# monahand1023/imageclust

Measured on AMD Instinct MI355X. Metric: images/sec (embed+Ward), higher is better.
Workload: dtype bf16; 1 GPU; the metric's size (configs[2]'s N=100000) on 1 GPU: 100000 synthetic 224x224x3 images (structured, seed 20250217; 100000 on this rank), ResNet50-v1 bf16 batch=256 -> 2048-d pooled E -> Ward min=5 max=50 (merge loop on GPU0) -> cluster ids on host; n_images_total=100000, embed_dim=2048, weights=synthetic seed 1, device=AMD Radeon Graphics (gfx950:sramecc+:xnack-)

## Files before the change

imageclust_amd/csrc/conv_p8.h:

```cpp
#pragma once
#include "mfma_tile.h"
#include "resnet_fused.h"

template <int MW, int NWV>
struct p8_geom {
    static_assert(MW * NWV == 8 && (NWV == 4 || NWV == 2), "8 waves");
    static constexpr int BM = MW * 128, BN = NWV * 64;
    static constexpr int PX = MW, PW = NWV / 2;
    static constexpr int SX = PX * 8192, SW = PW * 8192;
    static constexpr int O_WA = 0, O_XA = SW, O_WB = SW + SX, O_XB = 2 * SW + SX;
    static constexpr int BUF = 2 * (SW + SX);
    static constexpr int LDS = 2 * BUF;
    static constexpr int INFLIGHT = 2 * PW + PX;
    static_assert(INFLIGHT == 6 && LDS <= 160 * 1024, "counted vmcnt(6); the CU's 160 KiB");
};

template <int NP>
__device__ __forceinline__ void p8_dma(const i32x4_t &srd, const unsigned (&voff)[NP], unsigned soff, unsigned lds0)
{
    unsigned keep;
    if constexpr (NP == 1) {
        asm volatile("s_mov_b32 %0, m0\n\ts_mov_b32 m0, %4\n\ts_nop 4\n\tbuffer_load_dwordx4 %1, %2, %3 offen lds\n\ts_mov_b32 m0, %0"
                     : "=&s"(keep)
                     : "v"(voff[0]), "s"(srd), "s"(soff), "s"(lds0)
                     : "memory");
    } else if constexpr (NP == 2) {
        asm volatile("s_mov_b32 %0, m0\n\ts_mov_b32 m0, %5\n\ts_nop 4\n\tbuffer_load_dwordx4 %1, %3, %4 offen lds\n\t"
                     "s_mov_b32 m0, %6\n\ts_nop 0\n\tbuffer_load_dwordx4 %2, %3, %4 offen lds\n\ts_mov_b32 m0, %0"
                     : "=&s"(keep)
                     : "v"(voff[0]), "v"(voff[1]), "s"(srd), "s"(soff), "s"(lds0), "s"(lds0 + 0x2000u)
                     : "memory");
    } else {
        static_assert(NP == 4, "1, 2 or 4 pieces");
        asm volatile("s_mov_b32 %0, m0\n\ts_mov_b32 m0, %7\n\ts_nop 4\n\tbuffer_load_dwordx4 %1, %5, %6 offen lds\n\t"
                     "s_mov_b32 m0, %8\n\ts_nop 0\n\tbuffer_load_dwordx4 %2, %5, %6 offen lds\n\t"
                     "s_mov_b32 m0, %9\n\ts_nop 0\n\tbuffer_load_dwordx4 %3, %5, %6 offen lds\n\t"
                     "s_mov_b32 m0, %10\n\ts_nop 0\n\tbuffer_load_dwordx4 %4, %5, %6 offen lds\n\ts_mov_b32 m0, %0"
                     : "=&s"(keep)
                     : "v"(voff[0]), "v"(voff[1]), "v"(voff[2]), "v"(voff[3]), "s"(srd), "s"(soff), "s"(lds0), "s"(lds0 + 0x2000u), "s"(lds0 + 0x4000u),
                       "s"(lds0 + 0x6000u)
                     : "memory");
    }
}

template <int MW, int NWV, bool TAPS, bool DUAL, bool SPLIT = false, bool X3 = false>
__global__ __launch_bounds__(512) void conv_p8_kernel(const conv_args p)
{
    static_assert(!(SPLIT && DUAL), "the split form covers single-operand layers");
    static_assert(!(SPLIT && X3), "the split form is bf16 only");
    typedef p8_geom<MW, NWV> G;
    typedef unsigned u32x2_t __attribute__((ext_vector_type(2)));
    constexpr int PX = G::PX, PW = G::PW;
    __shared__ __attribute__((aligned(1024))) unsigned char smem[G::LDS];
    const int tid = threadIdx.x, lane = tid & 63;
    const int wid = __builtin_amdgcn_readfirstlane(tid >> 6);
    const int wr = wid / NWV, wc = wid % NWV;
    const int grp = wid >> 2;
    const int ntile = p.gx * p.gy;
    const int role = SPLIT ? (int)blockIdx.x / ntile : 0;
    const int tile = xcd_remap((int)blockIdx.x - role * ntile, ntile);
    const int m0 = (tile / p.gy) * G::BM, n0 = (tile % p.gy) * G::BN;
    const i32x4_t xsrd = bn56_srd(p.X, (unsigned)((size_t)p.B * p.H * p.W * p.Cin * 2));
    const i32x4_t wsrd = bn56_srd(p.Wt, (unsigned)((size_t)p.Cout * p.K * 2));
    const i32x4_t x2srd = DUAL ? bn56_srd(p.X2, (unsigned)((size_t)p.B * p.H2 * p.W2 * p.Cin2 * 2)) : xsrd;

    unsigned vx[2][PX], vw[2][PW], vx2[DUAL ? 2 : 1][PX], vmask[TAPS ? 2 : 1][PX];
#pragma unroll
    for (int j = 0; j < PX; ++j) {
        const int sr = (j * 8 + wid) * 8 + (lane >> 3);
        const unsigned ls16 = (unsigned)(((lane & 7) ^ ((sr >> 1) & 7)) << 4);
#pragma unroll
        for (int h = 0; h < 2; ++h) {
            const int m = m0 + (sr >> 6) * 128 + h * 64 + (sr & 63);
            const bool ok = (int64_t)m < p.M;
            const unsigned mm = ok ? (unsigned)m : 0u;
            const unsigned tq = mm / (unsigned)p.Wo;
            const int ox = (int)(mm - tq * (unsigned)p.Wo);
            const int b = (int)(tq / (unsigned)p.Ho);
            const int oy = (int)(tq - (unsigned)b * (unsigned)p.Ho);
            const int iy0 = oy * p.stride - p.pad, ix0 = ox * p.stride - p.pad;
            const unsigned off = (unsigned)((((b * p.H + iy0) * p.W + ix0) * p.Cin) * 2) + ls16;
            if (TAPS) {
                unsigned mk = 0;
                for (int kh = 0; kh < p.KH; ++kh)
                    for (int kw = 0; kw < p.KW; ++kw)
                        if (ok && (unsigned)(iy0 + kh) < (unsigned)p.H && (unsigned)(ix0 + kw) < (unsigned)p.W) mk |= 1u << (kh * p.KW + kw);
                vmask[h][j] = mk;
                vx[h][j] = off;
            } else {
                vx[h][j] = ok ? off : BN56_OOB;
            }
            if (DUAL) vx2[h][j] = ok ? (unsigned)((((b * p.H2 + oy * p.stride2) * p.W2 + ox * p.stride2) * p.Cin2) * 2) + ls16 : BN56_OOB;
        }
    }
#pragma unroll
    for (int j = 0; j < PW; ++j) {
        const int sr = (j * 8 + wid) * 8 + (lane >> 3);
        const unsigned ls16 = (unsigned)(((lane & 7) ^ ((sr >> 1) & 7)) << 4);
#pragma unroll
        for (int h = 0; h < 2; ++h) {
            const int wrow = n0 + (sr >> 5) * 64 + h * 32 + (sr & 31);
            vw[h][j] = (unsigned)wrow * (unsigned)p.K * 2u + ls16;
        }
    }
    const unsigned lds0 = __builtin_amdgcn_readfirstlane(lds_addr_of(smem) + wid * 1024);
    const int l15 = lane & 15, q = lane >> 4, fsw = (l15 >> 1) & 7;
    const unsigned char *xrd[2], *wrd[2];
#pragma unroll
    for (int s = 0; s < 2; ++s) {
        const int ph = ((4 * s + q) ^ fsw) << 4;
        xrd[s] = smem + (wr * 64 + l15) * 128 + ph;
        wrd[s] = smem + (wc * 32 + l15) * 128 + ph;
    }
    f32x4 acc[8][4];
#pragma unroll
    for (int i = 0; i < 8; ++i)
#pragma unroll
        for (int j = 0; j < 4; ++j) acc[i][j] = f32x4{0.f, 0.f, 0.f, 0.f};

    const int nt = SPLIT ? p.K / 128 : p.K / 64;
    const int kt0 = (SPLIT && role == 0) ? nt : 0;
    const int nt1 = (p.KH * p.KW * p.Cin) / 64;
    int xs_t = kt0, xs_ci = 0, xs_kw = 0, xs_kh = 0;
    unsigned xs_off = 0, xs_bit = 1;
    if (SPLIT && TAPS && kt0) {
        const int cpt = p.Cin / 64, tap = kt0 / cpt;
        xs_ci = (kt0 - tap * cpt) * 64;
        xs_kh = tap / p.KW;
        xs_kw = tap - xs_kh * p.KW;
        xs_bit = 1u << tap;
        xs_off = (unsigned)(((xs_kh * p.W + xs_kw) * p.Cin + xs_ci) * 2);
    }
    auto stage_w = [&](int h, int buf, int t) {
        p8_dma<PW>(wsrd, vw[h], (unsigned)(kt0 + t) * 128u, lds0 + buf * G::BUF + (h ? G::O_WB : G::O_WA));
    };
    auto stage_x = [&](int h, int buf) {
        const unsigned dst = lds0 + buf * G::BUF + (h ? G::O_XB : G::O_XA);
        if (DUAL && xs_t >= nt1) {
            p8_dma<PX>(x2srd, vx2[DUAL ? h : 0], (unsigned)(xs_t - nt1) * 128u, dst);
        } else if (TAPS) {
            unsigned v[PX];
#pragma unroll
            for (int j = 0; j < PX; ++j) v[j] = (vmask[TAPS ? h : 0][j] & xs_bit) ? vx[h][j] + xs_off : BN56_OOB;
            p8_dma<PX>(xsrd, v, 0u, dst);
        } else {
            p8_dma<PX>(xsrd, vx[h], (unsigned)xs_t * 128u, dst);
        }
        if (h == 1) {
            ++xs_t;
            if (TAPS) {
                xs_ci += 64;
                if (xs_ci == p.Cin) {
                    xs_ci = 0;
                    xs_bit <<= 1;
                    if (++xs_kw == p.KW) {
                        xs_kw = 0;
                        ++xs_kh;
                    }
                }
                xs_off = (unsigned)(((xs_kh * p.W + xs_kw) * p.Cin + xs_ci) * 2);
            }
        }
    };
    uint4 xf[4][2], w0[2][2], w1[2][2];
    auto mma = [&](int hx, int hw, uint4 (&wf)[2][2]) {
        __builtin_amdgcn_s_barrier();
        asm volatile("s_waitcnt lgkmcnt(0)" ::: "memory");
        __builtin_amdgcn_s_setprio(1);
        if constexpr (X3) {
#pragma unroll
            for (int u = 0; u < 3; ++u)
#pragma unroll
                for (int m = 0; m < 4; ++m)
#pragma unroll
                    for (int n = 0; n < 2; ++n) acc[hx * 4 + m][hw * 2 + n] = mfma16(wf[n][u == 1], xf[m][u == 2], acc[hx * 4 + m][hw * 2 + n]);
        } else {
#pragma unroll
            for (int s = 0; s < 2; ++s)
#pragma unroll
                for (int m = 0; m < 4; ++m)
#pragma unroll
                    for (int n = 0; n < 2; ++n) acc[hx * 4 + m][hw * 2 + n] = mfma16(wf[n][s], xf[m][s], acc[hx * 4 + m][hw * 2 + n]);
        }
        __builtin_amdgcn_s_setprio(0);
        __builtin_amdgcn_s_barrier();
    };
    auto ktile = [&](auto bufc, auto modec, int t) {
        constexpr int BUF = decltype(bufc)::value, MODE = decltype(modec)::value;
        const size_t bo = (size_t)BUF * G::BUF;
#pragma unroll
        for (int n = 0; n < 2; ++n)
#pragma unroll
            for (int s = 0; s < 2; ++s) w0[n][s] = *reinterpret_cast<const uint4 *>(wrd[s] + bo + G::O_WA + n * 2048);
        __builtin_amdgcn_sched_barrier(0);
#pragma unroll
        for (int m = 0; m < 4; ++m)
#pragma unroll
            for (int s = 0; s < 2; ++s) xf[m][s] = *reinterpret_cast<const uint4 *>(xrd[s] + bo + G::O_XA + m * 2048);
        if (MODE <= 1) stage_x(1, BUF ^ 1);
        asm volatile("s_waitcnt lgkmcnt(8)" ::: "memory");
        mma(0, 0, w0);
#pragma unroll
        for (int n = 0; n < 2; ++n)
#pragma unroll
            for (int s = 0; s < 2; ++s) w1[n][s] = *reinterpret_cast<const uint4 *>(wrd[s] + bo + G::O_WB + n * 2048);
        if (MODE == 0) stage_w(0, BUF, t + 2);
        mma(0, 1, w1);
#pragma unroll
        for (int m = 0; m < 4; ++m)
#pragma unroll
            for (int s = 0; s < 2; ++s) xf[m][s] = *reinterpret_cast<const uint4 *>(xrd[s] + bo + G::O_XB + m * 2048);
        if (MODE == 0) stage_x(0, BUF);
        mma(1, 1, w1);
        if (MODE == 0) {
            stage_w(1, BUF, t + 2);
            asm volatile("s_waitcnt vmcnt(6)" ::: "memory");
        } else if (MODE == 1) {
            asm volatile("s_waitcnt vmcnt(0)" ::: "memory");
        }
        mma(1, 0, w0);
    };
    stage_w(0, 0, 0);
    stage_x(0, 0);
    stage_w(1, 0, 0);
    stage_x(1, 0);
    stage_w(0, 1, 1);
    stage_x(0, 1);
    stage_w(1, 1, 1);
    asm volatile("s_waitcnt vmcnt(6)" ::: "memory");
    __builtin_amdgcn_s_barrier();
    if (grp == 1) __builtin_amdgcn_s_barrier();
    int t = 0;
    for (; t + 4 <= nt; t += 2) {
        ktile(std::integral_constant<int, 0>(), std::integral_constant<int, 0>(), t);
        ktile(std::integral_constant<int, 1>(), std::integral_constant<int, 0>(), t + 1);
    }
    ktile(std::integral_constant<int, 0>(), std::integral_constant<int, 1>(), t);
    ktile(std::integral_constant<int, 1>(), std::integral_constant<int, 2>(), t + 1);
    if (grp == 0) __builtin_amdgcn_s_barrier();

    if constexpr (SPLIT) {
        typedef unsigned u32x4_t __attribute__((ext_vector_type(4)));
        const __amdgpu_buffer_rsrc_t psrd = __builtin_amdgcn_make_buffer_rsrc(p.sk_part, 0, (int)((size_t)ntile * (32 * 512 * 16)), 0x00020000);
        const int voff = tid * 16;
        const int soff0 = tile * (32 * 512 * 16);
        if (role == 0) {
#pragma unroll
            for (int i = 0; i < 8; ++i)
#pragma unroll
                for (int j = 0; j < 4; ++j)
                    __builtin_amdgcn_raw_buffer_store_b128(__builtin_bit_cast(u32x4_t, acc[i][j]), psrd, voff, soff0 + (i * 4 + j) * 8192, 16 );
            asm volatile("s_waitcnt vmcnt(0)" ::: "memory");
            __syncthreads();
            if (tid == 0) __hip_atomic_store(p.sk_flag + tile, p.sk_epoch, __ATOMIC_RELAXED, __HIP_MEMORY_SCOPE_AGENT);
            return;
        }
        for (int spin = 0; spin < (1 << 22); ++spin) {
            if (__hip_atomic_load(p.sk_flag + tile, __ATOMIC_RELAXED, __HIP_MEMORY_SCOPE_AGENT) == p.sk_epoch) break;
            __builtin_amdgcn_s_sleep(2);
        }
        __builtin_amdgcn_fence(__ATOMIC_ACQUIRE, "wavefront");
#pragma unroll
        for (int g = 0; g < 4; ++g) {
            u32x4_t o[8];
#pragma unroll
            for (int k = 0; k < 8; ++k) o[k] = __builtin_amdgcn_raw_buffer_load_b128(psrd, voff, soff0 + (g * 8 + k) * 8192, 16 );
#pragma unroll
            for (int k = 0; k < 8; ++k) acc[(g * 8 + k) >> 2][(g * 8 + k) & 3] += __builtin_bit_cast(f32x4, o[k]);
        }
    }

    typedef uint16_t elem;
    elem *Yg = (elem *)p.Y;
    const elem *Rg = (const elem *)p.R;
    const int cbl = (q & 1) * 16 + (q >> 1) * 8;
    const int64_t yld = X3 ? 2 * (int64_t)p.Cout : (int64_t)p.Cout;
    auto ycol = [&](int c) { return X3 ? c + (c & ~31) : c; };
    float sc[2][8], sh[2][8];
#pragma unroll
    for (int i = 0; i < 2; ++i) {
        const int c = n0 + wc * 64 + i * 32 + cbl;
        const float4 a0 = *reinterpret_cast<const float4 *>(p.scale + c), a1 = *reinterpret_cast<const float4 *>(p.scale + c + 4);
        const float4 b0 = *reinterpret_cast<const float4 *>(p.shift + c), b1 = *reinterpret_cast<const float4 *>(p.shift + c + 4);
        sc[i][0] = a0.x; sc[i][1] = a0.y; sc[i][2] = a0.z; sc[i][3] = a0.w; sc[i][4] = a1.x; sc[i][5] = a1.y; sc[i][6] = a1.z; sc[i][7] = a1.w;
        sh[i][0] = b0.x; sh[i][1] = b0.y; sh[i][2] = b0.z; sh[i][3] = b0.w; sh[i][4] = b1.x; sh[i][5] = b1.y; sh[i][6] = b1.z; sh[i][7] = b1.w;
    }
#pragma unroll
    for (int hx = 0; hx < 2; ++hx) {
        uint4 rv[4][2], rl[2];
        if (Rg && !X3) {
#pragma unroll
            for (int m = 0; m < 4; ++m) {
                const int64_t mrow = (int64_t)m0 + wr * 128 + hx * 64 + m * 16 + l15;
#pragma unroll
                for (int i = 0; i < 2; ++i)
                    rv[m][i] = mrow < p.M ? *reinterpret_cast<const uint4 *>(Rg + mrow * p.Cout + n0 + wc * 64 + i * 32 + cbl) : make_uint4(0, 0, 0, 0);
            }
        }
#pragma unroll
        for (int m = 0; m < 4; ++m) {
            const int64_t mrow = (int64_t)m0 + wr * 128 + hx * 64 + m * 16 + l15;
            if (X3 && Rg) {
#pragma unroll
                for (int i = 0; i < 2; ++i) {
                    const elem *r = Rg + mrow * yld + ycol(n0 + wc * 64 + i * 32 + cbl);
                    rv[m][i] = mrow < p.M ? *reinterpret_cast<const uint4 *>(r) : make_uint4(0, 0, 0, 0);
                    rl[i] = mrow < p.M ? *reinterpret_cast<const uint4 *>(r + 32) : make_uint4(0, 0, 0, 0);
                }
            }
#pragma unroll
            for (int i = 0; i < 2; ++i) {
                const f32x4 ta = acc[hx * 4 + m][2 * i], tb = acc[hx * 4 + m][2 * i + 1];
                float v[8];
#pragma unroll
                for (int j = 0; j < 4; ++j) {
                    const u32x2_t r = __builtin_amdgcn_permlane16_swap(__float_as_uint(ta[j]), __float_as_uint(tb[j]), false, false);
                    v[j] = __uint_as_float(r[0]);
                    v[4 + j] = __uint_as_float(r[1]);
                }
#pragma unroll
                for (int e = 0; e < 8; ++e) v[e] = v[e] * sc[i][e] + sh[i][e];
                if (Rg) {
                    const elem *re = reinterpret_cast<const elem *>(&rv[m][i]);
                    if constexpr (X3) {
                        const elem *rle = reinterpret_cast<const elem *>(&rl[i]);
#pragma unroll
                        for (int e = 0; e < 8; ++e) v[e] += BF16::to_f(re[e]) + BF16::to_f(rle[e]);
                    } else {
#pragma unroll
                        for (int e = 0; e < 8; ++e) v[e] += BF16::to_f(re[e]);
                    }
                }
                if (p.relu) {
#pragma unroll
                    for (int e = 0; e < 8; ++e) v[e] = fmaxf(v[e], 0.0f);
                }
                uint4 ov, ol;
                elem *oe = reinterpret_cast<elem *>(&ov);
                if constexpr (X3) {
                    elem *ole = reinterpret_cast<elem *>(&ol);
#pragma unroll
                    for (int e = 0; e < 8; ++e) BF16X3::split(v[e], oe[e], ole[e]);
                } else {
#pragma unroll
                    for (int e = 0; e < 8; ++e) oe[e] = BF16::from_f(v[e]);
                }
                elem *yo = Yg + mrow * yld + ycol(n0 + wc * 64 + i * 32 + cbl);
                if (mrow < p.M) {
                    *reinterpret_cast<uint4 *>(yo) = ov;
                    if (X3) *reinterpret_cast<uint4 *>(yo + 32) = ol;
                }
            }
        }
    }
}

#ifndef P8_AUTO_MIN_NT
#define P8_AUTO_MIN_NT 4
#endif
static int conv_p8_layout(const conv_args &a) { return a.Cout % 256 == 0 ? 1 : (a.Cout % 128 == 0 ? 2 : 0); }
static bool conv_p8_eligible(const conv_args &a, int mode )
{
    if (mode == 0) return false;
    const int lay = conv_p8_layout(a);
    if (!lay || a.Cin % 64 || (a.X2 && a.Cin2 % 64)) return false;
    if (a.KH * a.KW > 9 || a.KH * a.KW * a.Cin + (a.X2 ? a.Cin2 : 0) != a.K) return false;
    if (a.X2 && (a.KH != 1 || a.KW != 1 || a.stride != 1 || a.pad != 0)) return false;
    const int nt = a.K / 64;
    if (a.K % 128) return false;
    if ((size_t)a.B * a.H * a.W * a.Cin * 2 >= (1ull << 31) || (size_t)a.Cout * a.K * 2 >= (1ull << 31)) return false;
    if (a.X2 && (size_t)a.B * a.H2 * a.W2 * a.Cin2 * 2 >= (1ull << 31)) return false;
    if (a.M >= (1ll << 31) - 512) return false;
    if (mode >= 2) return true;
    return nt >= P8_AUTO_MIN_NT;
}

static bool conv_p8_split_eligible(const icl_ctx *ctx, const conv_args &a)
{
    return ctx->conv_sk && !a.X2 && a.Ho * a.Wo <= 49 && a.K % 256 == 0 && a.K >= ctx->conv_sk_min_k && a.Cout % 256 == 0;
}
static int conv_p8_split_scratch(icl_ctx *ctx, hipStream_t strm, int tiles, conv_args &a)
{
    icl_sk_slot *sl = nullptr;
    for (auto &s : ctx->sk)
        if (s.part && s.stream == strm) sl = &s;
    if (!sl)
        for (auto &s : ctx->sk)
            if (!s.part && !sl) sl = &s;
    if (!sl) return ICL_ERR_NOMEM;
    if (sl->cap < tiles) {
        if (sl->part) {
            ICL_HIP(ctx, hipStreamSynchronize(strm));
            (void)hipFree(sl->part);
            (void)hipFree(sl->flag);
            sl->part = nullptr;
            sl->flag = nullptr;
            sl->cap = 0;
        }
        if (tiles > 4096) return ICL_ERR_UNSUPPORTED;
        const int cap = std::max(tiles, 128);
        ICL_HIP(ctx, hipMalloc(&sl->part, (size_t)cap * 32 * 512 * 16));
        ICL_HIP(ctx, hipMalloc((void **)&sl->flag, (size_t)cap * 4));
        ICL_HIP(ctx, hipMemsetAsync(sl->flag, 0, (size_t)cap * 4, strm));
        sl->cap = cap;
        sl->stream = strm;
        sl->epoch = 0;
    }
    a.sk_part = sl->part;
    a.sk_flag = sl->flag;
    a.sk_epoch = ++sl->epoch;
    return ICL_OK;
}

template <int MW, int NWV, bool X3>
static void launch_conv_p8_t(icl_ctx *ctx, conv_args &a)
{
    typedef p8_geom<MW, NWV> G;
    hipStream_t strm = ctx->cur_stream ? ctx->cur_stream : ctx->stream;
    a.gx = (int)icl_ceil_div(a.M, G::BM);
    a.gy = a.Cout / G::BN;
    const bool taps = a.KH * a.KW > 1 || a.pad != 0;
    if constexpr (NWV == 4 && !X3) {
        if (conv_p8_split_eligible(ctx, a) && conv_p8_split_scratch(ctx, strm, a.gx * a.gy, a) == ICL_OK) {
            const dim3 grid2((unsigned)(2 * a.gx * a.gy));
            if (taps) hipLaunchKernelGGL((conv_p8_kernel<MW, NWV, true, false, true>), grid2, dim3(512), 0, strm, a);
            else hipLaunchKernelGGL((conv_p8_kernel<MW, NWV, false, false, true>), grid2, dim3(512), 0, strm, a);
            ++ctx->conv_sk_launches;
            return;
        }
    }
    const dim3 grid((unsigned)(a.gx * a.gy));
    if (a.X2) hipLaunchKernelGGL((conv_p8_kernel<MW, NWV, false, true, false, X3>), grid, dim3(512), 0, strm, a);
    else if (taps) hipLaunchKernelGGL((conv_p8_kernel<MW, NWV, true, false, false, X3>), grid, dim3(512), 0, strm, a);
    else hipLaunchKernelGGL((conv_p8_kernel<MW, NWV, false, false, false, X3>), grid, dim3(512), 0, strm, a);
}
template <bool X3 = false>
static void launch_conv_p8(icl_ctx *ctx, conv_args &a)
{
    if (conv_p8_layout(a) == 1) launch_conv_p8_t<2, 4, X3>(ctx, a);
    else launch_conv_p8_t<4, 2, X3>(ctx, a);
}
```

imageclust_amd/csrc/distance_i8.hip:

```cpp
#include "icl_common.h"
#include "distance.h"
#include "mfma_tile.h"

#include <algorithm>
#include <cmath>
#include <type_traits>

typedef int di8_i32x4 __attribute__((ext_vector_type(4)));

#define DI8_OOB 0x80000000u
#define DI8_SLOT 16384
#define DI8_BUF 65536
#define DI8_WA 0
#define DI8_XA 1
#define DI8_WB 2
#define DI8_XB 3

__device__ __forceinline__ di8_i32x4 di8_srd(const void *base, unsigned bytes)
{
    const unsigned long long a = (unsigned long long)base;
    di8_i32x4 r;
    r.x = __builtin_amdgcn_readfirstlane((int)(unsigned)a);
    r.y = __builtin_amdgcn_readfirstlane((int)(unsigned)(a >> 32));
    r.z = __builtin_amdgcn_readfirstlane((int)bytes);
    r.w = 0x00020000;
    return r;
}
__device__ __forceinline__ void di8_dma2(const di8_i32x4 &srd, unsigned voff0, unsigned voff1, unsigned soff, unsigned lds0)
{
    unsigned keep;
    const unsigned lds1 = lds0 + 0x2000u;
    asm volatile("s_mov_b32 %0, m0\n\t"
                 "s_mov_b32 m0, %5\n\t"
                 "s_nop 4\n\t"
                 "buffer_load_dwordx4 %1, %3, %4 offen lds\n\t"
                 "s_mov_b32 m0, %6\n\t"
                 "s_nop 0\n\t"
                 "buffer_load_dwordx4 %2, %3, %4 offen lds\n\t"
                 "s_mov_b32 m0, %0"
                 : "=&s"(keep)
                 : "v"(voff0), "v"(voff1), "s"(srd), "s"(soff), "s"(lds0), "s"(lds1)
                 : "memory");
}
__device__ __forceinline__ di8_i32x4 di8_mfma(const uint4 &a, const uint4 &b, const di8_i32x4 &c)
{
    return __builtin_amdgcn_mfma_i32_16x16x64_i8(__builtin_bit_cast(di8_i32x4, a), __builtin_bit_cast(di8_i32x4, b), c, 0, 0, 0);
}

__global__ __launch_bounds__(256) void dist_quant_kernel(const float *__restrict__ Ec, int64_t n, int K, int Kp, int8_t *__restrict__ Q,
                                                        int32_t *__restrict__ ex, float *__restrict__ l1)
{
    __shared__ float red[2][4];
    const int64_t r = blockIdx.x;
    if (r >= n) return;
    const float *row = Ec + r * K;
    float mx = 0.0f, sum = 0.0f;
    bool bad = false;
    for (int k = threadIdx.x; k < K; k += 256) {
        const float a = fabsf(row[k]);
        bad |= !(a < 3.0e38f);
        mx = fmaxf(mx, a);
        sum += a;
    }
#pragma unroll
    for (int off = 32; off > 0; off >>= 1) {
        mx = fmaxf(mx, __shfl_down(mx, off, 64));
        sum += __shfl_down(sum, off, 64);
    }
    const bool anybad = __syncthreads_or(bad ? 1 : 0) != 0;
    if ((threadIdx.x & 63) == 0) {
        red[0][threadIdx.x >> 6] = mx;
        red[1][threadIdx.x >> 6] = sum;
    }
    __syncthreads();
    mx = fmaxf(fmaxf(red[0][0], red[0][1]), fmaxf(red[0][2], red[0][3]));
    sum = (red[1][0] + red[1][1]) + (red[1][2] + red[1][3]);
    int e = 0;
    const bool zero = anybad || !(mx > 0.0f);
    if (!zero) (void)frexpf(mx, &e);
    if (threadIdx.x == 0) {
        ex[r] = zero ? INT32_MIN : e;
        l1[r] = zero ? 0.0f : sum * (1.0f + 2.0f * (float)K * 5.9604645e-8f) * 1.000001f;
    }
    int8_t *q = Q + r * 3 * (int64_t)Kp;
    for (int k = threadIdx.x; k < Kp; k += 256) {
        int q1 = 0, q2 = 0, q3 = 0;
        if (!zero && k < K) {
            const int A = (int)rint(ldexp((double)row[k], 20 - e));
            q3 = ((A + 64) & 127) - 64;
            const int A1 = (A - q3) >> 7;
            q2 = ((A1 + 64) & 127) - 64;
            q1 = (A1 - q2) >> 7;
        }
        q[k] = (int8_t)q1;
        q[Kp + k] = (int8_t)q2;
        q[2 * Kp + k] = (int8_t)q3;
    }
}

struct di8_args {
    const int8_t *Q;
    const float *nrm, *l1;
    const int32_t *ex;
    float *out;
    const int64_t *rowoff;
    int64_t n;
    int T;
    int Kp, d;
    float gam;
    unsigned int *rowub;
};

__device__ __forceinline__ double di8_eab(double sa, double sb, double l1a, double l1b, double na, double nb, int d)
{
    const double t21 = 4.76837158203125e-07;
    const double m = t21 * (sa * (l1b + (double)d * sb * t21) + sb * l1a) + sa * sb * (double)d * (1048576.0 + 4096.0) * 9.094947017729282e-13;
    return (m + 16.0 * 5.9604644775390625e-08 * (1.0 + 64.0 * 5.9604644775390625e-08) * (na + nb)) * (1.0 + 1e-12);
}

__global__ __launch_bounds__(512) void dist_bound_i8_kernel(const di8_args p)
{
    __shared__ __attribute__((aligned(1024))) unsigned char smem[2 * DI8_BUF];
    const int tid = threadIdx.x, lane = tid & 63;
    const int wid = __builtin_amdgcn_readfirstlane(tid >> 6);
    const int wr = wid >> 2, wc = wid & 3;
    int ti, tj;
    tri_band_decode(xcd_remap((int)blockIdx.x, (int)gridDim.x), 0, p.T, ti, tj);
    ti = __builtin_amdgcn_readfirstlane(ti);
    tj = __builtin_amdgcn_readfirstlane(tj);
    const int64_t m0 = (int64_t)ti * 256, n0 = (int64_t)tj * 256;
    const unsigned rowb = 3u * (unsigned)p.Kp;
    const int64_t xrows = p.n - m0 < 256 ? p.n - m0 : 256, wrows = p.n - n0 < 256 ? p.n - n0 : 256;
    const di8_i32x4 asrd = di8_srd(p.Q + m0 * (int64_t)rowb, (unsigned)xrows * rowb), bsrd = di8_srd(p.Q + n0 * (int64_t)rowb, (unsigned)wrows * rowb);
    unsigned vx[2][2], vw[2][2];
#pragma unroll
    for (int j = 0; j < 2; ++j) {
        const int sr = (j * 8 + wid) * 8 + (lane >> 3);
        const int ls = (lane & 7) ^ ((sr >> 1) & 7);
#pragma unroll
        for (int h = 0; h < 2; ++h) {
            const int xr = (sr >> 6) * 128 + h * 64 + (sr & 63);
            const int wrow = (sr >> 5) * 64 + h * 32 + (sr & 31);
            vx[h][j] = xr < xrows ? (unsigned)xr * rowb + ls * 16u : DI8_OOB;
            vw[h][j] = wrow < wrows ? (unsigned)wrow * rowb + ls * 16u : DI8_OOB;
        }
    }
    const unsigned lds0 = __builtin_amdgcn_readfirstlane(lds_addr_of(smem) + wid * 1024);
    const int l15 = lane & 15, q = lane >> 4, f = (l15 >> 1) & 7;
    const unsigned char *xrd[2], *wrd[2];
#pragma unroll
    for (int s = 0; s < 2; ++s) {
        const int ph = ((4 * s + q) ^ f) << 4;
        xrd[s] = smem + (wr * 64 + l15) * 128 + ph;
        wrd[s] = smem + (wc * 32 + l15) * 128 + ph;
    }
    di8_i32x4 acc[8][4];
#pragma unroll
    for (int i = 0; i < 8; ++i)
#pragma unroll
        for (int j = 0; j < 4; ++j) acc[i][j] = di8_i32x4{0, 0, 0, 0};

    const int nt = 6 * p.Kp / 128, b1 = p.Kp / 128, b2 = 3 * p.Kp / 128;
    auto stage = [&](int slot, int buf, int t) {
        const unsigned dst = __builtin_amdgcn_readfirstlane(lds0 + buf * DI8_BUF + slot * DI8_SLOT);
        const int pr = (t >= b1) + (t >= 2 * b1) + (t >= 3 * b1) + (t >= 4 * b1) + (t >= 5 * b1);
        const bool isx = slot == DI8_XA || slot == DI8_XB;
        const unsigned dig = ((isx ? 0x120100u : 0x102010u) >> (4 * pr)) & 15u;
        const unsigned soff = __builtin_amdgcn_readfirstlane(dig * (unsigned)p.Kp + (unsigned)(t - pr * b1) * 128u);
        if (slot == DI8_WA) di8_dma2(bsrd, vw[0][0], vw[0][1], soff, dst);
        else if (slot == DI8_WB) di8_dma2(bsrd, vw[1][0], vw[1][1], soff, dst);
        else if (slot == DI8_XA) di8_dma2(asrd, vx[0][0], vx[0][1], soff, dst);
        else di8_dma2(asrd, vx[1][0], vx[1][1], soff, dst);
    };
    uint4 xf[4][2], w0[2][2], w1[2][2];
    auto mma = [&](int hx, int hw, uint4 (&wf)[2][2]) {
        __builtin_amdgcn_s_barrier();
        asm volatile("s_waitcnt lgkmcnt(0)" ::: "memory");
        __builtin_amdgcn_s_setprio(1);
#pragma unroll
        for (int s = 0; s < 2; ++s)
#pragma unroll
            for (int m = 0; m < 4; ++m)
#pragma unroll
                for (int n = 0; n < 2; ++n) acc[hx * 4 + m][hw * 2 + n] = di8_mfma(wf[n][s], xf[m][s], acc[hx * 4 + m][hw * 2 + n]);
        __builtin_amdgcn_s_setprio(0);
        __builtin_amdgcn_s_barrier();
    };
    auto ktile = [&](auto bufc, auto modec, int t) {
        constexpr int BUF = decltype(bufc)::value, MODE = decltype(modec)::value;
        const size_t bo = (size_t)BUF * DI8_BUF;
#pragma unroll
        for (int n = 0; n < 2; ++n)
#pragma unroll
            for (int s = 0; s < 2; ++s) w0[n][s] = *reinterpret_cast<const uint4 *>(wrd[s] + bo + DI8_WA * DI8_SLOT + n * 2048);
        __builtin_amdgcn_sched_barrier(0);
#pragma unroll
        for (int m = 0; m < 4; ++m)
#pragma unroll
            for (int s = 0; s < 2; ++s) xf[m][s] = *reinterpret_cast<const uint4 *>(xrd[s] + bo + DI8_XA * DI8_SLOT + m * 2048);
        if (MODE <= 1) stage(DI8_XB, BUF ^ 1, t + 1);
        asm volatile("s_waitcnt lgkmcnt(8)" ::: "memory");
        mma(0, 0, w0);
#pragma unroll
        for (int n = 0; n < 2; ++n)
#pragma unroll
            for (int s = 0; s < 2; ++s) w1[n][s] = *reinterpret_cast<const uint4 *>(wrd[s] + bo + DI8_WB * DI8_SLOT + n * 2048);
        if (MODE == 0) stage(DI8_WA, BUF, t + 2);
        mma(0, 1, w1);
#pragma unroll
        for (int m = 0; m < 4; ++m)
#pragma unroll
            for (int s = 0; s < 2; ++s) xf[m][s] = *reinterpret_cast<const uint4 *>(xrd[s] + bo + DI8_XB * DI8_SLOT + m * 2048);
        if (MODE == 0) stage(DI8_XA, BUF, t + 2);
        mma(1, 1, w1);
        if (MODE == 0) {
            stage(DI8_WB, BUF, t + 2);
            asm volatile("s_waitcnt vmcnt(6)" ::: "memory");
        } else if (MODE == 1) {
            asm volatile("s_waitcnt vmcnt(0)" ::: "memory");
        }
        mma(1, 0, w0);
    };
    auto out_ptr = [&](int mt, int ntl, int64_t &i, int64_t &j) -> float * {
        i = m0 + wr * 128 + (mt >> 2) * 64 + (mt & 3) * 16 + l15;
        j = n0 + wc * 64 + (ntl >> 1) * 32 + (ntl & 1) * 16 + 4 * q;
        return i < p.n ? p.out + p.rowoff[i] + j : nullptr;
    };
    stage(DI8_WA, 0, 0);
    stage(DI8_XA, 0, 0);
    stage(DI8_WB, 0, 0);
    stage(DI8_XB, 0, 0);
    stage(DI8_WA, 1, 1);
    stage(DI8_XA, 1, 1);
    stage(DI8_WB, 1, 1);
    asm volatile("s_waitcnt vmcnt(6)" ::: "memory");
    __builtin_amdgcn_s_barrier();
    if (wr == 1) __builtin_amdgcn_s_barrier();
    int t = 0;
    for (; t + 4 <= nt; t += 2) {
        if (t == b1) {
#pragma unroll
            for (int i = 0; i < 8; ++i)
#pragma unroll
                for (int j = 0; j < 4; ++j) acc[i][j] = acc[i][j] * 128;
        }
        if (t == b2) {
#pragma unroll
            for (int mt = 0; mt < 8; ++mt)
#pragma unroll
                for (int ntl = 0; ntl < 4; ++ntl) {
                    int64_t i, j;
                    float *o = out_ptr(mt, ntl, i, j);
                    if (o && j < i) {
                        *reinterpret_cast<di8_i32x4 *>(o) = acc[mt][ntl];
                    }
                    acc[mt][ntl] = di8_i32x4{0, 0, 0, 0};
                }
            asm volatile("s_waitcnt vmcnt(0)" ::: "memory");
        }
        ktile(std::integral_constant<int, 0>(), std::integral_constant<int, 0>(), t);
        ktile(std::integral_constant<int, 1>(), std::integral_constant<int, 0>(), t + 1);
    }
    ktile(std::integral_constant<int, 0>(), std::integral_constant<int, 1>(), t);
    ktile(std::integral_constant<int, 1>(), std::integral_constant<int, 2>(), t + 1);
    if (wr == 0) __builtin_amdgcn_s_barrier();
    float um[8];
#pragma unroll
    for (int mt = 0; mt < 8; ++mt) um[mt] = ICL_MAXF;
#pragma unroll
    for (int ntl = 0; ntl < 4; ++ntl) {
        const int64_t j = n0 + wc * 64 + (ntl >> 1) * 32 + (ntl & 1) * 16 + 4 * q;
        double sj[4], l1j[4], nj[4];
#pragma unroll
        for (int e = 0; e < 4; ++e) {
            const bool in = j + e < p.n;
            const int ej = in ? p.ex[j + e] : INT32_MIN;
            sj[e] = ej == INT32_MIN ? 0.0 : ldexp(1.0, ej);
            l1j[e] = in ? (double)p.l1[j + e] : 0.0;
            nj[e] = in ? (double)p.nrm[j + e] : 0.0;
        }
#pragma unroll
        for (int mt = 0; mt < 8; ++mt) {
            const int64_t i = m0 + wr * 128 + (mt >> 2) * 64 + (mt & 3) * 16 + l15;
            if (i >= p.n || j >= i) continue;
            const int ei = p.ex[i];
            const double si = ei == INT32_MIN ? 0.0 : ldexp(1.0, ei), l1i = (double)p.l1[i], ni = (double)p.nrm[i];
            float *row = p.out + p.rowoff[i];
            const di8_i32x4 hi = *reinterpret_cast<const di8_i32x4 *>(row + j);
            float v[4];
#pragma unroll
            for (int e = 0; e < 4; ++e) {
                const double I = 128.0 * (double)hi[e] + (double)acc[mt][ntl][e];
                const double c = si * sj[e] * 1.4901161193847656e-08 * I;
                const double ns = ni + nj[e];
                const double T = 0.5 * ns - c;
                const double Eab = di8_eab(si, sj[e], l1i, l1j[e], ni, nj[e], p.d);
                const double Ld = (T - Eab) * (1.0 - (double)p.gam) * (1.0 - 1e-12);
                const float L = (Ld > 1e-30 && ns < 1e37) ? __double2float_rz(Ld) : 0.0f;
                v[e] = __uint_as_float(__float_as_uint(L) | 0x80000000u);
                if (j + e < i) {
                    const double U = ((double)L * (1.0 + 3.0 * (double)p.gam) + 2.0001 * Eab + 2e-30) * (1.0 + 2.0 * (double)p.gam);
                    const float Uf = U < 3.0e38 ? __double2float_ru(U) : ICL_MAXF;
                    um[mt] = fminf(um[mt], Uf);
                }
            }
            if (j + 3 < i) {
                *reinterpret_cast<float4 *>(row + j) = make_float4(v[0], v[1], v[2], v[3]);
            } else {
#pragma unroll
                for (int e = 0; e < 4; ++e)
                    if (j + e < i) row[j + e] = v[e];
            }
        }
    }
    if (p.rowub) {
#pragma unroll
        for (int mt = 0; mt < 8; ++mt) {
            float u = um[mt];
            u = fminf(u, __shfl_xor(u, 16, 64));
            u = fminf(u, __shfl_xor(u, 32, 64));
            const int64_t i = m0 + wr * 128 + (mt >> 2) * 64 + (mt & 3) * 16 + l15;
            if (q == 0 && i < p.n && u < ICL_MAXF) atomicMin(&p.rowub[i], __float_as_uint(u));
        }
    }
}

bool icl_dist_i8_usable(int64_t n, int d) { return d >= 1 && d <= 2048 && n < (1LL << 29); }
size_t icl_dist_i8_pq_bytes(int64_t n, int d)
{
    const int64_t Kp = (d + 255) / 256 * 256;
    return (size_t)(n * 3 * Kp) + 256;
}

int icl_dist_bound_i8_launch(icl_ctx *ctx, const float *d_Ec, const float *d_nrm, int64_t n, int d, int K, float gam, void *d_pq, float *d_l1, int32_t *d_ex,
                             float *d_out, const int64_t *d_rowoff, hipStream_t strm, unsigned int *d_rowub)
{
    const int Kp = (d + 255) / 256 * 256;
    int8_t *Q = reinterpret_cast<int8_t *>(d_pq);
    if (n <= 0) return ICL_OK;
    hipLaunchKernelGGL(dist_quant_kernel, dim3((unsigned)n), dim3(256), 0, strm, d_Ec, n, K, Kp, Q, d_ex, d_l1);
    const int64_t T = icl_ceil_div(n, 256);
    int64_t nblocks;
    ICL_TRY(icl_dist_grid(ctx, 0, T, &nblocks));
    if (d_rowub) ICL_HIP(ctx, hipMemsetAsync(d_rowub, 0x7f, (size_t)n * sizeof(unsigned int), strm));
    di8_args a{Q, d_nrm, d_l1, d_ex, d_out, d_rowoff, n, (int)T, Kp, d, gam, d_rowub};
    const double pairs = 0.5 * (double)n * (double)(n - 1);
    icl_prof_scope ps(ctx, ICL_K_DIST_MFMA, 2.0 * pairs * 6.0 * Kp, 4.0 * pairs + (double)n * 3.0 * Kp);
    hipLaunchKernelGGL(dist_bound_i8_kernel, dim3((unsigned)nblocks), dim3(512), 0, strm, a);
    ICL_HIP(ctx, hipGetLastError());
    return ICL_OK;
}
```

Measured before the change: 70900 images/sec.

## Overlap conv address setup with DMA, specialize interior epilogues in conv and int8 distance

The conv kernel now computes each half's X row addresses just before staging it, so the first weight DMAs go out earlier. It builds the tap-validity masks arithmetically instead of with nested loops, packs both halves into one mask register, and prefetches the BN scale and shift during the last k-tile. Conv and int8-distance epilogues gain interior-tile specializations that skip bounds checks. The distance epilogue also hoists per-row loads and moves the bound math into a shared header; it adds code size and register pressure.

```diff
diff --git a/imageclust_amd/csrc/conv_p8.h b/imageclust_amd/csrc/conv_p8.h
--- a/imageclust_amd/csrc/conv_p8.h
+++ b/imageclust_amd/csrc/conv_p8.h
@@ -64,13 +64,26 @@
     const i32x4_t wsrd = bn56_srd(p.Wt, (unsigned)((size_t)p.Cout * p.K * 2));
     const i32x4_t x2srd = DUAL ? bn56_srd(p.X2, (unsigned)((size_t)p.B * p.H2 * p.W2 * p.Cin2 * 2)) : xsrd;
 
-    unsigned vx[2][PX], vw[2][PW], vx2[DUAL ? 2 : 1][PX], vmask[TAPS ? 2 : 1][PX];
-#pragma unroll
-    for (int j = 0; j < PX; ++j) {
+    unsigned vx[2][PX], vw[2][PW], vx2[DUAL ? 2 : 1][PX], vmask[PX];
+#pragma unroll
+    for (int j = 0; j < PW; ++j) {
         const int sr = (j * 8 + wid) * 8 + (lane >> 3);
         const unsigned ls16 = (unsigned)(((lane & 7) ^ ((sr >> 1) & 7)) << 4);
 #pragma unroll
         for (int h = 0; h < 2; ++h) {
+            const int wrow = n0 + (sr >> 5) * 64 + h * 32 + (sr & 31);
+            vw[h][j] = (unsigned)wrow * (unsigned)p.K * 2u + ls16;
+        }
+    }
+    const unsigned lds0 = __builtin_amdgcn_readfirstlane(lds_addr_of(smem) + wid * 1024);
+    unsigned taprep = 0;
+    if (TAPS)
+        for (int kh = 0; kh < p.KH; ++kh) taprep |= 1u << (kh * p.KW);
+    auto xrows = [&](int h) {
+#pragma unroll
+        for (int j = 0; j < PX; ++j) {
+            const int sr = (j * 8 + wid) * 8 + (lane >> 3);
+            const unsigned ls16 = (unsigned)(((lane & 7) ^ ((sr >> 1) & 7)) << 4);
             const int m = m0 + (sr >> 6) * 128 + h * 64 + (sr & 63);
             const bool ok = (int64_t)m < p.M;
             const unsigned mm = ok ? (unsigned)m : 0u;
@@ -81,42 +94,19 @@
             const int iy0 = oy * p.stride - p.pad, ix0 = ox * p.stride - p.pad;
             const unsigned off = (unsigned)((((b * p.H + iy0) * p.W + ix0) * p.Cin) * 2) + ls16;
             if (TAPS) {
-                unsigned mk = 0;
-                for (int kh = 0; kh < p.KH; ++kh)
-                    for (int kw = 0; kw < p.KW; ++kw)
-                        if (ok && (unsigned)(iy0 + kh) < (unsigned)p.H && (unsigned)(ix0 + kw) < (unsigned)p.W) mk |= 1u << (kh * p.KW + kw);
-                vmask[h][j] = mk;
+                const int c0 = std::min(std::max(-ix0, 0), p.KW), c1 = std::min(std::max(p.W - ix0, 0), p.KW);
+                const int r0 = std::min(std::max(-iy0, 0), p.KH), r1 = std::min(std::max(p.H - iy0, 0), p.KH);
+                const unsigned cols = ((1u << (c1 - c0)) - 1u) << c0;
+                const unsigned rows = ((1u << ((r1 - r0) * p.KW)) - 1u) << (r0 * p.KW);
+                const unsigned mk = ok ? (cols * taprep) & rows : 0u;
+                vmask[j] = h ? vmask[j] | (mk << 16) : mk;
                 vx[h][j] = off;
             } else {
                 vx[h][j] = ok ? off : BN56_OOB;
             }
-            if (DUAL) vx2[h][j] = ok ? (unsigned)((((b * p.H2 + oy * p.stride2) * p.W2 + ox * p.stride2) * p.Cin2) * 2) + ls16 : BN56_OOB;
-        }
-    }
-#pragma unroll
-    for (int j = 0; j < PW; ++j) {
-        const int sr = (j * 8 + wid) * 8 + (lane >> 3);
-        const unsigned ls16 = (unsigned)(((lane & 7) ^ ((sr >> 1) & 7)) << 4);
-#pragma unroll
-        for (int h = 0; h < 2; ++h) {
-            const int wrow = n0 + (sr >> 5) * 64 + h * 32 + (sr & 31);
-            vw[h][j] = (unsigned)wrow * (unsigned)p.K * 2u + ls16;
-        }
-    }
-    const unsigned lds0 = __builtin_amdgcn_readfirstlane(lds_addr_of(smem) + wid * 1024);
-    const int l15 = lane & 15, q = lane >> 4, fsw = (l15 >> 1) & 7;
-    const unsigned char *xrd[2], *wrd[2];
-#pragma unroll
-    for (int s = 0; s < 2; ++s) {
-        const int ph = ((4 * s + q) ^ fsw) << 4;
-        xrd[s] = smem + (wr * 64 + l15) * 128 + ph;
-        wrd[s] = smem + (wc * 32 + l15) * 128 + ph;
-    }
-    f32x4 acc[8][4];
-#pragma unroll
-    for (int i = 0; i < 8; ++i)
-#pragma unroll
-        for (int j = 0; j < 4; ++j) acc[i][j] = f32x4{0.f, 0.f, 0.f, 0.f};
+            if (DUAL) vx2[DUAL ? h : 0][j] = ok ? (unsigned)((((b * p.H2 + oy * p.stride2) * p.W2 + ox * p.stride2) * p.Cin2) * 2) + ls16 : BN56_OOB;
+        }
+    };
 
     const int nt = SPLIT ? p.K / 128 : p.K / 64;
     const int kt0 = (SPLIT && role == 0) ? nt : 0;
@@ -139,9 +129,10 @@
         if (DUAL && xs_t >= nt1) {
             p8_dma<PX>(x2srd, vx2[DUAL ? h : 0], (unsigned)(xs_t - nt1) * 128u, dst);
         } else if (TAPS) {
+            const unsigned bit = h ? xs_bit << 16 : xs_bit;
             unsigned v[PX];
 #pragma unroll
-            for (int j = 0; j < PX; ++j) v[j] = (vmask[TAPS ? h : 0][j] & xs_bit) ? vx[h][j] + xs_off : BN56_OOB;
+            for (int j = 0; j < PX; ++j) v[j] = (vmask[j] & bit) ? vx[h][j] + xs_off : BN56_OOB;
             p8_dma<PX>(xsrd, v, 0u, dst);
         } else {
             p8_dma<PX>(xsrd, vx[h], (unsigned)xs_t * 128u, dst);
@@ -162,6 +153,43 @@
             }
         }
     };
+    stage_w(0, 0, 0);
+    __builtin_amdgcn_sched_barrier(0);
+    xrows(0);
+    stage_x(0, 0);
+    stage_w(1, 0, 0);
+    __builtin_amdgcn_sched_barrier(0);
+    xrows(1);
+    stage_x(1, 0);
+    stage_w(0, 1, 1);
+    stage_x(0, 1);
+    stage_w(1, 1, 1);
+    __builtin_amdgcn_sched_barrier(0);
+    const int l15 = lane & 15, q = lane >> 4, fsw = (l15 >> 1) & 7;
+    const unsigned char *xrd[2], *wrd[2];
+#pragma unroll
+    for (int s = 0; s < 2; ++s) {
+        const int ph = ((4 * s + q) ^ fsw) << 4;
+        xrd[s] = smem + (wr * 64 + l15) * 128 + ph;
+        wrd[s] = smem + (wc * 32 + l15) * 128 + ph;
+    }
+    f32x4 acc[8][4];
+#pragma unroll
+    for (int i = 0; i < 8; ++i)
+#pragma unroll
+        for (int j = 0; j < 4; ++j) acc[i][j] = f32x4{0.f, 0.f, 0.f, 0.f};
+    float4 sc4[2][2], sh4[2][2];
+    auto load_affine = [&]() {
+        const int cb = n0 + wc * 64 + (q & 1) * 16 + (q >> 1) * 8;
+#pragma unroll
+        for (int i = 0; i < 2; ++i) {
+            sc4[i][0] = *reinterpret_cast<const float4 *>(p.scale + cb + i * 32);
+            sc4[i][1] = *reinterpret_cast<const float4 *>(p.scale + cb + i * 32 + 4);
+            sh4[i][0] = *reinterpret_cast<const float4 *>(p.shift + cb + i * 32);
+            sh4[i][1] = *reinterpret_cast<const float4 *>(p.shift + cb + i * 32 + 4);
+        }
+    };
+
     uint4 xf[4][2], w0[2][2], w1[2][2];
     auto mma = [&](int hx, int hw, uint4 (&wf)[2][2]) {
         __builtin_amdgcn_s_barrier();
@@ -188,6 +216,7 @@
     auto ktile = [&](auto bufc, auto modec, int t) {
         constexpr int BUF = decltype(bufc)::value, MODE = decltype(modec)::value;
         const size_t bo = (size_t)BUF * G::BUF;
+        if constexpr (MODE == 2 && !SPLIT && !X3) load_affine();
 #pragma unroll
         for (int n = 0; n < 2; ++n)
 #pragma unroll
@@ -220,13 +249,6 @@
         }
         mma(1, 0, w0);
     };
-    stage_w(0, 0, 0);
-    stage_x(0, 0);
-    stage_w(1, 0, 0);
-    stage_x(1, 0);
-    stage_w(0, 1, 1);
-    stage_x(0, 1);
-    stage_w(1, 1, 1);
     asm volatile("s_waitcnt vmcnt(6)" ::: "memory");
     __builtin_amdgcn_s_barrier();
     if (grp == 1) __builtin_amdgcn_s_barrier();
@@ -270,21 +292,23 @@
         }
     }
 
+    if constexpr (SPLIT || X3) load_affine();
     typedef uint16_t elem;
+    const int cbl = (q & 1) * 16 + (q >> 1) * 8;
     elem *Yg = (elem *)p.Y;
     const elem *Rg = (const elem *)p.R;
-    const int cbl = (q & 1) * 16 + (q >> 1) * 8;
     const int64_t yld = X3 ? 2 * (int64_t)p.Cout : (int64_t)p.Cout;
     auto ycol = [&](int c) { return X3 ? c + (c & ~31) : c; };
     float sc[2][8], sh[2][8];
 #pragma unroll
     for (int i = 0; i < 2; ++i) {
-        const int c = n0 + wc * 64 + i * 32 + cbl;
-        const float4 a0 = *reinterpret_cast<const float4 *>(p.scale + c), a1 = *reinterpret_cast<const float4 *>(p.scale + c + 4);
-        const float4 b0 = *reinterpret_cast<const float4 *>(p.shift + c), b1 = *reinterpret_cast<const float4 *>(p.shift + c + 4);
+        const float4 a0 = sc4[i][0], a1 = sc4[i][1], b0 = sh4[i][0], b1 = sh4[i][1];
         sc[i][0] = a0.x; sc[i][1] = a0.y; sc[i][2] = a0.z; sc[i][3] = a0.w; sc[i][4] = a1.x; sc[i][5] = a1.y; sc[i][6] = a1.z; sc[i][7] = a1.w;
         sh[i][0] = b0.x; sh[i][1] = b0.y; sh[i][2] = b0.z; sh[i][3] = b0.w; sh[i][4] = b1.x; sh[i][5] = b1.y; sh[i][6] = b1.z; sh[i][7] = b1.w;
     }
+    auto epilogue = [&](auto fullc) {
+    constexpr bool FULL = decltype(fullc)::value;
+    auto inside = [&](int64_t mrow) { return FULL || mrow < p.M; };
 #pragma unroll
     for (int hx = 0; hx < 2; ++hx) {
         uint4 rv[4][2], rl[2];
@@ -294,7 +318,7 @@
                 const int64_t mrow = (int64_t)m0 + wr * 128 + hx * 64 + m * 16 + l15;
 #pragma unroll
                 for (int i = 0; i < 2; ++i)
-                    rv[m][i] = mrow < p.M ? *reinterpret_cast<const uint4 *>(Rg + mrow * p.Cout + n0 + wc * 64 + i * 32 + cbl) : make_uint4(0, 0, 0, 0);
+                    rv[m][i] = inside(mrow) ? *reinterpret_cast<const uint4 *>(Rg + mrow * p.Cout + n0 + wc * 64 + i * 32 + cbl) : make_uint4(0, 0, 0, 0);
             }
         }
 #pragma unroll
@@ -304,8 +328,8 @@
 #pragma unroll
                 for (int i = 0; i < 2; ++i) {
                     const elem *r = Rg + mrow * yld + ycol(n0 + wc * 64 + i * 32 + cbl);
-                    rv[m][i] = mrow < p.M ? *reinterpret_cast<const uint4 *>(r) : make_uint4(0, 0, 0, 0);
-                    rl[i] = mrow < p.M ? *reinterpret_cast<const uint4 *>(r + 32) : make_uint4(0, 0, 0, 0);
+                    rv[m][i] = inside(mrow) ? *reinterpret_cast<const uint4 *>(r) : make_uint4(0, 0, 0, 0);
+                    rl[i] = inside(mrow) ? *reinterpret_cast<const uint4 *>(r + 32) : make_uint4(0, 0, 0, 0);
                 }
             }
 #pragma unroll
@@ -346,13 +370,16 @@
                     for (int e = 0; e < 8; ++e) oe[e] = BF16::from_f(v[e]);
                 }
                 elem *yo = Yg + mrow * yld + ycol(n0 + wc * 64 + i * 32 + cbl);
-                if (mrow < p.M) {
+                if (inside(mrow)) {
                     *reinterpret_cast<uint4 *>(yo) = ov;
                     if (X3) *reinterpret_cast<uint4 *>(yo + 32) = ol;
                 }
             }
         }
     }
+    };
+    if (!X3 && !SPLIT && (int64_t)m0 + G::BM <= p.M) epilogue(std::true_type());
+    else epilogue(std::false_type());
 }
 
 #ifndef P8_AUTO_MIN_NT
diff --git a/imageclust_amd/csrc/dist_i8_bound.h b/imageclust_amd/csrc/dist_i8_bound.h
--- /dev/null
+++ b/imageclust_amd/csrc/dist_i8_bound.h
@@ -0,0 +1,81 @@
+#pragma once
+#include <cmath>
+#include <cstdint>
+#include <cstring>
+
+#if defined(__HIPCC__) || defined(__CUDACC__)
+#define DI8B_HD __host__ __device__ __forceinline__
+#else
+#define DI8B_HD inline
+#endif
+
+#define DI8B_NOEXP INT32_MIN
+#define DI8B_MAXF 3.40282346638528859811704183484516925e+38f
+
+DI8B_HD double di8_kappa() { return 16.0 * 5.9604644775390625e-08 * (1.0 + 64.0 * 5.9604644775390625e-08); }
+
+DI8B_HD double di8_pow2(int e)
+{
+    const uint64_t bits = e == DI8B_NOEXP ? 0ull : (uint64_t)(unsigned)(e + 1023) << 52;
+    double s;
+    memcpy(&s, &bits, sizeof s);
+    return s;
+}
+
+struct di8_side {
+    double s, s26, p, k, n;
+};
+DI8B_HD di8_side di8_side_of(int e, float l1, float nrm)
+{
+    di8_side r;
+    r.s = di8_pow2(e);
+    r.s26 = r.s * 1.4901161193847656e-08;
+    r.p = (double)l1 * 4.76837158203125e-07;
+    r.n = (double)nrm;
+    r.k = di8_kappa() * r.n;
+    return r;
+}
+
+DI8B_HD double di8_cd(int d) { return (double)d * 2.2737367544323206e-13 + (double)d * (1048576.0 + 4096.0) * 9.094947017729282e-13; }
+
+DI8B_HD double di8_eab(const di8_side &a, const di8_side &b, double cd)
+{
+    return (a.s * b.p + b.s * a.p + (a.s * b.s) * cd + (a.k + b.k)) * (1.0 + 1e-12);
+}
+
+DI8B_HD double di8_T(const di8_side &a, const di8_side &b, double I) { return 0.5 * (a.n + b.n) - (a.s26 * b.s) * I; }
+
+DI8B_HD float di8_f32_rz_pos(double v)
+{
+    const float f = (float)v;
+    uint32_t u;
+    memcpy(&u, &f, sizeof u);
+    u -= (double)f > v ? 1u : 0u;
+    float r;
+    memcpy(&r, &u, sizeof r);
+    return r;
+}
+DI8B_HD float di8_f32_ru_pos(double v)
+{
+    const float f = (float)v;
+    uint32_t u;
+    memcpy(&u, &f, sizeof u);
+    u += (double)f < v ? 1u : 0u;
+    float r;
+    memcpy(&r, &u, sizeof r);
+    return r;
+}
+
+DI8B_HD float di8_lower(double T, double Eab, double ns, double gam)
+{
+    const double Ld = (T - Eab) * (1.0 - gam) * (1.0 - 1e-12);
+    const float L = di8_f32_rz_pos(Ld);
+    return (Ld > 1e-30 && ns < 1e37) ? L : 0.0f;
+}
+
+DI8B_HD float di8_upper(float L, double Eab, double gam)
+{
+    const double U = ((double)L * (1.0 + 3.0 * gam) + 2.0001 * Eab + 2e-30) * (1.0 + 2.0 * gam);
+    const float Uf = di8_f32_ru_pos(U);
+    return U < 3.0e38 ? Uf : DI8B_MAXF;
+}
diff --git a/imageclust_amd/csrc/distance_i8.hip b/imageclust_amd/csrc/distance_i8.hip
--- a/imageclust_amd/csrc/distance_i8.hip
+++ b/imageclust_amd/csrc/distance_i8.hip
@@ -1,5 +1,6 @@
 #include "icl_common.h"
 #include "distance.h"
+#include "dist_i8_bound.h"
 #include "mfma_tile.h"
 
 #include <algorithm>
@@ -111,13 +112,6 @@
     unsigned int *rowub;
 };
 
-__device__ __forceinline__ double di8_eab(double sa, double sb, double l1a, double l1b, double na, double nb, int d)
-{
-    const double t21 = 4.76837158203125e-07;
-    const double m = t21 * (sa * (l1b + (double)d * sb * t21) + sb * l1a) + sa * sb * (double)d * (1048576.0 + 4096.0) * 9.094947017729282e-13;
-    return (m + 16.0 * 5.9604644775390625e-08 * (1.0 + 64.0 * 5.9604644775390625e-08) * (na + nb)) * (1.0 + 1e-12);
-}
-
 __global__ __launch_bounds__(512) void dist_bound_i8_kernel(const di8_args p)
 {
     __shared__ __attribute__((aligned(1024))) unsigned char smem[2 * DI8_BUF];
@@ -264,65 +258,86 @@
     ktile(std::integral_constant<int, 0>(), std::integral_constant<int, 1>(), t);
     ktile(std::integral_constant<int, 1>(), std::integral_constant<int, 2>(), t + 1);
     if (wr == 0) __builtin_amdgcn_s_barrier();
-    float um[8];
-#pragma unroll
-    for (int mt = 0; mt < 8; ++mt) um[mt] = ICL_MAXF;
-#pragma unroll
-    for (int ntl = 0; ntl < 4; ++ntl) {
-        const int64_t j = n0 + wc * 64 + (ntl >> 1) * 32 + (ntl & 1) * 16 + 4 * q;
-        double sj[4], l1j[4], nj[4];
-#pragma unroll
-        for (int e = 0; e < 4; ++e) {
-            const bool in = j + e < p.n;
-            const int ej = in ? p.ex[j + e] : INT32_MIN;
-            sj[e] = ej == INT32_MIN ? 0.0 : ldexp(1.0, ej);
-            l1j[e] = in ? (double)p.l1[j + e] : 0.0;
-            nj[e] = in ? (double)p.nrm[j + e] : 0.0;
-        }
+    const double cd = di8_cd(p.d), gam = (double)p.gam;
+    auto epilogue = [&](auto interiorc) {
+        constexpr bool INTERIOR = decltype(interiorc)::value;
+        float *rptr[8];
+        float um[8];
 #pragma unroll
         for (int mt = 0; mt < 8; ++mt) {
             const int64_t i = m0 + wr * 128 + (mt >> 2) * 64 + (mt & 3) * 16 + l15;
-            if (i >= p.n || j >= i) continue;
-            const int ei = p.ex[i];
-            const double si = ei == INT32_MIN ? 0.0 : ldexp(1.0, ei), l1i = (double)p.l1[i], ni = (double)p.nrm[i];
-            float *row = p.out + p.rowoff[i];
-            const di8_i32x4 hi = *reinterpret_cast<const di8_i32x4 *>(row + j);
-            float v[4];
+            rptr[mt] = (INTERIOR || i < p.n) ? p.out + p.rowoff[i] : nullptr;
+            um[mt] = ICL_MAXF;
+        }
+#pragma unroll
+        for (int ntl = 0; ntl < 4; ++ntl) {
+            const int64_t j = n0 + wc * 64 + (ntl >> 1) * 32 + (ntl & 1) * 16 + 4 * q;
+            di8_side cb[4];
 #pragma unroll
             for (int e = 0; e < 4; ++e) {
-                const double I = 128.0 * (double)hi[e] + (double)acc[mt][ntl][e];
-                const double c = si * sj[e] * 1.4901161193847656e-08 * I;
-                const double ns = ni + nj[e];
-                const double T = 0.5 * ns - c;
-                const double Eab = di8_eab(si, sj[e], l1i, l1j[e], ni, nj[e], p.d);
-                const double Ld = (T - Eab) * (1.0 - (double)p.gam) * (1.0 - 1e-12);
-                const float L = (Ld > 1e-30 && ns < 1e37) ? __double2float_rz(Ld) : 0.0f;
-                v[e] = __uint_as_float(__float_as_uint(L) | 0x80000000u);
-                if (j + e < i) {
-                    const double U = ((double)L * (1.0 + 3.0 * (double)p.gam) + 2.0001 * Eab + 2e-30) * (1.0 + 2.0 * (double)p.gam);
-                    const float Uf = U < 3.0e38 ? __double2float_ru(U) : ICL_MAXF;
-                    um[mt] = fminf(um[mt], Uf);
+                const bool in = INTERIOR || j + e < p.n;
+                cb[e] = di8_side_of(in ? p.ex[j + e] : DI8B_NOEXP, in ? p.l1[j + e] : 0.0f, in ? p.nrm[j + e] : 0.0f);
+            }
+#pragma unroll
+            for (int hx = 0; hx < 2; ++hx) {
+                di8_i32x4 hi[4];
+                int rex[4];
+                float rl1[4], rnr[4];
+                asm volatile("" ::: "memory");
+#pragma unroll
+                for (int m = 0; m < 4; ++m) {
+                    const int64_t i = m0 + wr * 128 + hx * 64 + m * 16 + l15;
+                    const bool live = INTERIOR || (i < p.n && j < i);
+                    hi[m] = live ? *reinterpret_cast<const di8_i32x4 *>(rptr[hx * 4 + m] + j) : di8_i32x4{0, 0, 0, 0};
+                    rex[m] = live ? p.ex[i] : DI8B_NOEXP;
+                    rl1[m] = live ? p.l1[i] : 0.0f;
+                    rnr[m] = live ? p.nrm[i] : 0.0f;
+                }
+#pragma unroll
+                for (int m = 0; m < 4; ++m) {
+                    const int mt = hx * 4 + m;
+                    const int64_t i = m0 + wr * 128 + hx * 64 + m * 16 + l15;
+                    if (!INTERIOR && (i >= p.n || j >= i)) continue;
+                    di8_i32x4 lo = acc[mt][ntl], hw = hi[m];
+                    asm volatile("" : "+v"(rex[m]), "+v"(rl1[m]), "+v"(rnr[m]), "+v"(lo), "+v"(hw)::"memory");
+                    const di8_side ra = di8_side_of(rex[m], rl1[m], rnr[m]);
+                    float v[4];
+#pragma unroll
+                    for (int e = 0; e < 4; ++e) {
+                        const double I = 128.0 * (double)hw[e] + (double)lo[e];
+                        const double Eab = di8_eab(ra, cb[e], cd);
+                        const float L = di8_lower(di8_T(ra, cb[e], I), Eab, ra.n + cb[e].n, gam);
+                        v[e] = __uint_as_float(__float_as_uint(L) | 0x80000000u);
+                        if (INTERIOR || j + e < i) um[mt] = fminf(um[mt], di8_upper(L, Eab, gam));
+                    }
+                    asm volatile("" : "+v"(um[mt]));
+                    if (INTERIOR || j + 3 < i) {
+                        *reinterpret_cast<float4 *>(rptr[mt] + j) = make_float4(v[0], v[1], v[2], v[3]);
+                    } else {
+#pragma unroll
+                        for (int e = 0; e < 4; ++e)
+                            if (j + e < i) rptr[mt][j + e] = v[e];
+                    }
                 }
             }
-            if (j + 3 < i) {
-                *reinterpret_cast<float4 *>(row + j) = make_float4(v[0], v[1], v[2], v[3]);
-            } else {
-#pragma unroll
-                for (int e = 0; e < 4; ++e)
-                    if (j + e < i) row[j + e] = v[e];
+        }
+        if (p.rowub) {
+#pragma unroll
+            for (int mt = 0; mt < 8; ++mt) {
+                um[mt] = fminf(um[mt], __shfl_xor(um[mt], 16, 64));
+                um[mt] = fminf(um[mt], __shfl_xor(um[mt], 32, 64));
             }
-        }
-    }
-    if (p.rowub) {
-#pragma unroll
-        for (int mt = 0; mt < 8; ++mt) {
-            float u = um[mt];
-            u = fminf(u, __shfl_xor(u, 16, 64));
-            u = fminf(u, __shfl_xor(u, 32, 64));
-            const int64_t i = m0 + wr * 128 + (mt >> 2) * 64 + (mt & 3) * 16 + l15;
-            if (q == 0 && i < p.n && u < ICL_MAXF) atomicMin(&p.rowub[i], __float_as_uint(u));
-        }
-    }
+            if (q == 0) {
+#pragma unroll
+                for (int mt = 0; mt < 8; ++mt) {
+                    const int64_t i = m0 + wr * 128 + (mt >> 2) * 64 + (mt & 3) * 16 + l15;
+                    if (INTERIOR || (i < p.n && um[mt] < ICL_MAXF)) atomicMin(&p.rowub[i], __float_as_uint(um[mt]));
+                }
+            }
+        }
+    };
+    if (tj < ti && m0 + 256 <= p.n) epilogue(std::true_type());
+    else epilogue(std::false_type());
 }
 
 bool icl_dist_i8_usable(int64_t n, int d) { return d >= 1 && d <= 2048 && n < (1LL << 29); }
```

Result: faster. 71940 images/sec, median of 6 (+1.5%).
